# lanl-ansi/GraphicalModelLearning.jl

Measured on AMD Instinct MI355X. Metric: obj/grad evals/sec (RISE, n=1024 spins, 1000000 samples), higher is better.
Workload: dtype i8w

## Files before the change

### graphicalmodellearning.jl_amd/csrc/gml_kernels_i8w.hip

```cpp
#include "gml_i8.h"
#include <string>
#include <type_traits>

namespace gml {

namespace {

constexpr int LFA = 4, LFB = 3;
constexpr int BRT = 32 * LFW;
constexpr int PA = 2 + 2 * LFA, PB = 2 + 2 * LFB;
constexpr int STEPW = PA * 1024, DSW = 2, STAGEW = DSW * STEPW, NSW = 3, RINGW = NSW * STAGEW;
constexpr int NLA = DSW * PA / 4, NLB = DSW * PB / 4;
static_assert(NLA == NLB + 1, "issue() drops the last load in sweep B");

__device__ __forceinline__ double flip_if(double v, int mneg ) {
    return __hiloint2double(__double2hiint(v) + (mneg << 31), __double2loint(v));
}

__device__ __forceinline__ void digits6(double yr, unsigned &dl, unsigned &dh) {
    unsigned long long v = ((unsigned long long)(unsigned)__double2hiint(yr) << 32) | (unsigned)__double2loint(yr);
    v += 0x0000808080808080ull;
    v ^= 0x0000808080808080ull;
    dl = (unsigned)v;
    dh = (unsigned)(v >> 32);
}

__device__ __forceinline__ void dma16(const int8_t *ubase, int voff, unsigned lds_addr) {
    asm volatile("s_mov_b32 m0, %2\n\ts_nop 0\n\tglobal_load_lds_dwordx4 %0, %1" ::"v"(voff), "s"(ubase), "s"(lds_addr) : "memory");
}

}

template <int FORM , bool WANTF, bool WIDE , bool UNIW,
          bool COARSE >
__global__ __launch_bounds__(256, 2) void k_fwd_i8w(
    const unsigned *__restrict__ Xb, const unsigned *__restrict__ Sb, const int8_t *__restrict__ Tq, const int *__restrict__ rowcol,
    const int *__restrict__ groups, int ngroups, const double *__restrict__ w, const double *__restrict__ sigma,
    const long long *__restrict__ qconst, const long long *__restrict__ qconst2, const double *__restrict__ invtau, int64_t Kp, int ntiles_k,
    int nk_all ,
    double wuni, int64_t Kreal, int8_t *__restrict__ Vq, long long *__restrict__ csum, long long *__restrict__ csum2,
    long long *__restrict__ asum, long long *__restrict__ asum2, double *__restrict__ fsum, unsigned *__restrict__ mmax,
    const int *__restrict__ cnk, const int8_t *__restrict__ Xc, int64_t xc_tile, int nk_tq) {
    constexpr int WM = 2;
    extern __shared__ __attribute__((aligned(16))) int8_t lds[];
    double *etab = reinterpret_cast<double *>(lds + RINGW);

    const int tid = threadIdx.x, wave = __builtin_amdgcn_readfirstlane(tid >> 6), lane = tid & 63;
    const int lr = lane & 31, h = lane >> 5;
    if (tid < 64) {
        const double v = exp2((double)tid / 64.0);
        etab[tid] = FORM == 0 ? __hiloint2double(__double2hiint(v) - (tid << 14), __double2loint(v)) : v;
    }
    if (FORM == 2 && tid < 64) {
        const double cj = 1.0 + ((double)tid + 0.5) / 64.0;
        etab[64 + tid] = 1.0 / cj;
        etab[128 + tid] = log(cj);
    }
    __syncthreads();

    constexpr int TG = 8;
    const int b = blockIdx.x, xcd = b & 7, bi = b >> 3;
    const int ntk8 = (ntiles_k + 7) >> 3;
    const int nfull = ngroups / TG, per_full = ntk8 * TG;
    int st, gi;
    if (bi < nfull * per_full) {
        const int rem = bi % per_full;
        st = (rem / TG) * 8 + xcd;
        gi = (bi / per_full) * TG + rem % TG;
    } else {
        const int lastn = ngroups - nfull * TG, rem = bi - nfull * per_full;
        st = (rem / lastn) * 8 + xcd;
        gi = nfull * TG + rem % lastn;
    }
    if (st >= ntiles_k) return;
    const int64_t k0 = (int64_t)st * 256;
    if (k0 >= Kp) return;
    const int mytile = groups[gi];
    int nk = nk_all;
    const int8_t *xbase = reinterpret_cast<const int8_t *>(Xb);
    if (cnk) {
        const int ck = cnk[mytile];
        if (ck >= 0) {
            nk = ck;
            xbase = Xc + (int64_t)mytile * xc_tile;
        }
    }

    const int voffX = lane * 16;
    const int voffT = (lane >> 2) * 64 + (((lane & 3) ^ ((lane >> 4) & 3)) << 4);
    const int8_t *const gX = xbase + (int64_t)(2 * st) * nk * 1024;
    const int8_t *const gT = Tq + (int64_t)mytile * nk_tq * BRT * 64;
    const int nst = (nk + DSW - 1) / DSW;
    const int8_t *baseA[NLA], *baseB[NLB];
    int advA[NLA], advB[NLB], subA[NLA], subB[NLB], dstA[NLA], dstB[NLB];
    bool bitsA[NLA], bitsB[NLB];
    auto plan = [&](int sp, int pps, int row0, const int8_t *&base, int &adv, int &sub, int &dst, bool &bits) {
        sub = sp / pps;
        const int pc = sp - sub * pps;
        dst = sub * STEPW + pc * 1024;
        bits = pc < 2;
        base = bits ? gX + (int64_t)pc * nk * 1024 : gT + (row0 + (pc - 2) * 16) * 64;
        adv = bits ? 1024 : BRT * 64;
    };
#pragma unroll
    for (int j = 0; j < NLA; ++j) plan(wave + 4 * j, PA, 32 * LFB, baseA[j], advA[j], subA[j], dstA[j], bitsA[j]);
#pragma unroll
    for (int j = 0; j < NLB; ++j) plan(wave + 4 * j, PB, 0, baseB[j], advB[j], subB[j], dstB[j], bitsB[j]);
    const unsigned lds0 = (unsigned)(uintptr_t)(__attribute__((address_space(3))) int8_t *)lds;
    auto issue = [&](int gs) {
        const unsigned stage_base = lds0 + (gs % NSW) * STAGEW;
        if (gs < nst) {
#pragma unroll
            for (int j = 0; j < NLA; ++j) {
                int kt = DSW * gs + subA[j];
                kt = kt < nk ? kt : nk - 1;
                dma16(baseA[j] + (int64_t)(kt * advA[j]), bitsA[j] ? voffX : voffT, stage_base + dstA[j]);
            }
        } else {
#pragma unroll
            for (int j = 0; j < NLB; ++j) {
                int kt = DSW * (gs - nst) + subB[j];
                kt = kt < nk ? kt : nk - 1;
                dma16(baseB[j] + (int64_t)(kt * advB[j]), bitsB[j] ? voffX : voffT, stage_base + dstB[j]);
            }
        }
    };

    const int r = mytile * 32 + lr;
    const int rc = rowcol[r];
    const bool active = rc >= 0;
    const double sg = active ? sigma[r] : 0.0;
    const long long qc = active ? (COARSE ? qconst2[r] : qconst[r]) : 0;
    const double c_lo = COARSE ? 0.0 : (double)(unsigned)(qc & 0xffffffll), c_hi = COARSE ? (double)qc : (double)(qc >> 24);
    const double sgT = sg * 16777216.0, us0 = c_hi * sgT, m2sT = -2.0 * sgT;
#ifdef ABL_EARLY_INPUTS
    unsigned sgn[WM];
#pragma unroll
    for (int i = 0; i < WM; ++i) sgn[i] = active ? (Sb[(int64_t)rc * (Kp >> 5) + ((k0 + wave * 64) >> 5) + i] >> (4 * h)) : 0u;
    const double it = active ? invtau[r] : 0.0;
#endif

#ifdef ABL_TIMING
    unsigned long long tst[6];
    tst[0] = __builtin_amdgcn_s_memrealtime();
#endif
    __builtin_amdgcn_s_setprio(1);
    const int ntot = COARSE ? nst : 2 * nst;
#pragma unroll
    for (int s = 0; s < NSW - 1; ++s)
        if (s < ntot) issue(s);
    auto gemm_stage = [&](int gs, int ks, auto first, auto &acc) {
        constexpr bool FIRST = decltype(first)::value;
        constexpr int NPL = sizeof(acc[0]) / sizeof(acc[0][0]);
        if (gs + 1 < ntot) {
            if (gs + 1 < nst) asm volatile("s_waitcnt vmcnt(%0)" ::"n"(NLA) : "memory");
            else asm volatile("s_waitcnt vmcnt(%0)" ::"n"(NLB) : "memory");
        } else {
            asm volatile("s_waitcnt vmcnt(0)" ::: "memory");
        }
        __builtin_amdgcn_s_barrier();
        __builtin_amdgcn_sched_barrier(0);
        if (gs + NSW - 1 < ntot) issue(gs + NSW - 1);
#pragma unroll
        for (int sub = 0; sub < DSW; ++sub) {
            if (sub > 0 && DSW * ks + sub >= nk) break;
            const int8_t *cur = lds + (gs % NSW) * STAGEW + sub * STEPW;
            unsigned vb[WM];
#pragma unroll
            for (int i = 0; i < WM; ++i) {
                const int row = wave * 64 + i * 32 + lr;
                vb[i] = *reinterpret_cast<const unsigned *>(cur + (row >> 7) * 1024 + (((row & 127) * 2 + h) << 2));
            }
#pragma unroll
            for (int t = 0; t < 2; ++t) {
                v4i fa[WM], fb[NPL];
#pragma unroll
                for (int l = 0; l < NPL; ++l) fb[l] = *reinterpret_cast<const v4i *>(cur + 2048 + lds_off(l * 32 + lr, 2 * t + h));
#pragma unroll
                for (int i = 0; i < WM; ++i)
#pragma unroll
                    for (int e = 0; e < 4; ++e) fa[i][e] = (int)((vb[i] >> (4 * t + e)) & 0x01010101u);
#pragma unroll
                for (int i = 0; i < WM; ++i)
#pragma unroll
                    for (int l = 0; l < NPL; ++l) {
                        if (FIRST && sub == 0 && t == 0) acc[i][l] = MFMA_I8(fa[i], fb[l], ((v16i){0, 0, 0, 0, 0, 0, 0, 0, 0, 0, 0, 0, 0, 0, 0, 0}));
                        else acc[i][l] = MFMA_I8(fa[i], fb[l], acc[i][l]);
                    }
            }
        }
    };

    double us[WM][16];
    {
        v16i acc[WM][LFA];
        if (nk > 0) {
            gemm_stage(0, 0, std::true_type{}, acc);
            for (int ks = 1; ks < nst; ++ks) gemm_stage(ks, ks, std::false_type{}, acc);
        } else {
#pragma unroll
            for (int i = 0; i < WM; ++i)
#pragma unroll
                for (int l = 0; l < LFA; ++l)
#pragma unroll
                    for (int e = 0; e < 16; ++e) acc[i][l][e] = 0;
        }
#ifdef ABL_TIMING
        tst[1] = __builtin_amdgcn_s_memrealtime();
#endif
#pragma unroll
        for (int i = 0; i < WM; ++i)
#pragma unroll
            for (int e = 0; e < 16; ++e) {
                double ahi;
                if (WIDE) {
                    ahi = (double)acc[i][3][e];
#pragma unroll
                    for (int l = 2; l >= 0; --l) ahi = fma(ahi, 256.0, (double)acc[i][l][e]);
                } else {
                    const int p0 = acc[i][0][e] + (acc[i][1][e] << 8), p1 = acc[i][2][e] + (acc[i][3][e] << 8);
                    ahi = fma((double)p1, 65536.0, (double)p0);
                }
                us[i][e] = fma(ahi, m2sT, us0);
                asm volatile("" : "+v"(us[i][e]));
            }
    }
#ifdef ABL_TIMING
    tst[2] = __builtin_amdgcn_s_memrealtime();
#endif
    if constexpr (!COARSE) {
        v16i acc[WM][LFB];
        if (nk > 0) {
            gemm_stage(nst, 0, std::true_type{}, acc);
#ifndef ABL_ONESWEEP
            for (int ks = 1; ks < nst; ++ks) gemm_stage(nst + ks, ks, std::false_type{}, acc);
#else
            asm volatile("s_waitcnt vmcnt(0)" ::: "memory");
#endif
        } else {
#pragma unroll
            for (int i = 0; i < WM; ++i)
#pragma unroll
                for (int l = 0; l < LFB; ++l)
#pragma unroll
                    for (int e = 0; e < 16; ++e) acc[i][l][e] = 0;
        }
#pragma unroll
        for (int i = 0; i < WM; ++i)
#pragma unroll
            for (int e = 0; e < 16; ++e) {
                double alo;
                if (WIDE) {
                    alo = fma((double)acc[i][2][e], 256.0, (double)acc[i][1][e]);
                    alo = fma(alo, 256.0, (double)acc[i][0][e]);
                } else {
                    alo = fma((double)acc[i][2][e], 65536.0, (double)(acc[i][0][e] + (acc[i][1][e] << 8)));
                }
                us[i][e] = fma(fma(alo, -2.0, c_lo), sg, us[i][e]);
            }
        __builtin_amdgcn_sched_barrier(0);
    }
    __builtin_amdgcn_s_setprio(0);
#ifdef ABL_TIMING
    tst[3] = __builtin_amdgcn_s_memrealtime();
#endif

#ifndef ABL_EARLY_INPUTS
    unsigned sgn[WM];
#pragma unroll
    for (int i = 0; i < WM; ++i) sgn[i] = active ? (Sb[(int64_t)rc * (Kp >> 5) + ((k0 + wave * 64) >> 5) + i] >> (4 * h)) : 0u;
    const double it = active ? invtau[r] : 0.0;
#endif
    const int64_t left = Kreal - (k0 + wave * 64 + 4 * h);
    const int nreal = left > 64 ? 64 : (left < 0 ? 0 : (int)left);

    int8_t *vimg = Vq + vq_off(mytile * 32 + lr, 0, k0 + wave * 64, Kp, LBW) + h * 32;
    const int64_t kw = k0 + wave * 64;
    const double wscale = COARSE ? 256.0 : 4294967296.0;
    const double wk32 = wscale * (wuni * it);
    const unsigned dh0 = (unsigned)rc * 0x85EBCA6Bu + (unsigned)(kw + 4 * h) * 0x9E3779B9u;
    constexpr double MAGIC = 6755399441055744.0, MAGIC32 = 6755399441055744.0 * 4294967296.0;
    constexpr unsigned GOLD = 0x9E3779B9u;
    const int wleft = (int)((Kreal - kw) < 64 ? (Kreal - kw) : 64);
    int csl[LBW] = {0, 0, 0, 0, 0, 0};
    unsigned long long as64 = 0;
    int ymax_hi = 0;
    double fp = 0.0;

    auto pack4 = [&](const unsigned (&dl)[4], const unsigned (&dhh)[4], v4i (&pl)[LBW], int slot) {
        if (COARSE) {
#pragma unroll
            for (int lb = 0; lb < 3; ++lb) {
                const unsigned sel = ((4u + lb) << 8) | (unsigned)lb;
                const unsigned pk = __builtin_amdgcn_perm(__builtin_amdgcn_perm(dl[3], dl[2], sel), __builtin_amdgcn_perm(dl[1], dl[0], sel), 0x05040100u);
                pl[3 + lb][slot] = (int)pk;
                csl[3 + lb] = __builtin_amdgcn_sdot4((int)pk, 0x01010101, csl[3 + lb], false);
            }
            pl[2][slot] = 0;
            return;
        }
#pragma unroll
        for (int lb = 0; lb < LBW; ++lb) {
            const unsigned bsel = (unsigned)(lb & 3);
            const unsigned sel = ((4u + bsel) << 8) | bsel;
            const unsigned t01 = lb < 4 ? __builtin_amdgcn_perm(dl[1], dl[0], sel) : __builtin_amdgcn_perm(dhh[1], dhh[0], sel);
            const unsigned t23 = lb < 4 ? __builtin_amdgcn_perm(dl[3], dl[2], sel) : __builtin_amdgcn_perm(dhh[3], dhh[2], sel);
            const unsigned pk = __builtin_amdgcn_perm(t23, t01, 0x05040100u);
            pl[lb][slot] = (int)pk;
            csl[lb] = __builtin_amdgcn_sdot4((int)pk, 0x01010101, csl[lb], false);
        }
    };

    if constexpr (FORM == 0) {
#define SB __builtin_amdgcn_sched_barrier(0)
#ifdef I8W_LINE_STORES
        v4i plk[WM][LBW];
#endif
#pragma unroll
        for (int i = 0; i < WM; ++i) {
            const unsigned nsg = ~sgn[i];
            v4i pl[LBW];
#pragma unroll
            for (int hg = 0; hg < 2; ++hg) {
                double Ea[8], tm[8], x[8], tj0[8], yy[8], pp[8], wk[8];
                int mneg[8], nn[8];
#pragma unroll
                for (int q = 0; q < 8; ++q) {
                    const int pos = 8 * (2 * hg + (q >> 2)) + (q & 3);
                    Ea[q] = us[i][8 * hg + q];
                    asm("v_bfe_i32 %0, %1, %2, 1" : "=v"(mneg[q]) : "v"(nsg), "n"(pos));
                    if (!UNIW) wk[q] = w[kw + i * 32 + 8 * (2 * hg + (q >> 2)) + 4 * h + (q & 3)];
                }
                SB;
#ifdef ABL_NOEPI
#pragma unroll
                for (int q = 0; q < 8; ++q) yy[q] = fma(fabs(Ea[q]), 1.0e21, 2.0e23);
                if (false) {
#endif
#pragma unroll
                for (int q = 0; q < 8; ++q) {
                    x[q] = flip_if(Ea[q], mneg[q]);
                    tm[q] = fma(x[q], 92.33248261689366, MAGIC);
                }
                SB;
#pragma unroll
                for (int q = 0; q < 8; ++q) {
                    nn[q] = __double2loint(tm[q]);
                    tm[q] = tm[q] - MAGIC;
                    tj0[q] = etab[nn[q] & 63];
                }
                SB;
#pragma unroll
                for (int q = 0; q < 8; ++q) x[q] = fma(tm[q], -0.01083042469326756, x[q]);
                SB;
#pragma unroll
                for (int q = 0; q < 8; ++q) x[q] = fma(tm[q], -2.9815858269852933e-12, x[q]);
                SB;
#pragma unroll
                for (int q = 0; q < 8; ++q) pp[q] = fma(x[q], 8.3333333333333332e-03, 4.1666666666666664e-02);
                SB;
#pragma unroll
                for (int q = 0; q < 8; ++q) pp[q] = fma(pp[q], x[q], 1.6666666666666666e-01);
                SB;
#pragma unroll
                for (int q = 0; q < 8; ++q) pp[q] = fma(pp[q], x[q], 0.5);
                SB;
#pragma unroll
                for (int q = 0; q < 8; ++q) pp[q] = fma(pp[q], x[q], 1.0);
                SB;
#pragma unroll
                for (int q = 0; q < 8; ++q) pp[q] = pp[q] * x[q];
                SB;
#pragma unroll
                for (int q = 0; q < 8; ++q) {
                    const int idx = i * 32 + 8 * (2 * hg + (q >> 2)) + (q & 3);
                    tj0[q] = __hiloint2double((int)((unsigned)__double2hiint(tj0[q]) + ((unsigned)nn[q] << 14)), __double2loint(tj0[q]));
                    yy[q] = (double)(int)(dh0 + (unsigned)idx * GOLD);
                }
                SB;
#pragma unroll
                for (int q = 0; q < 8; ++q) x[q] = fma(tj0[q], pp[q], tj0[q]);
                SB;
#pragma unroll
                for (int q = 0; q < 8; ++q) yy[q] = fma(UNIW ? wk32 : wscale * (wk[q] * it), x[q], yy[q]);
#ifdef ABL_NOEPI
                }
#endif
                if (UNIW && wleft < 64) {
                    asm volatile("; padding samples" ::: "memory");
#pragma unroll
                    for (int q = 0; q < 8; ++q)
                        if (i * 32 + 8 * (2 * hg + (q >> 2)) + (q & 3) >= nreal) yy[q] = 0.0;
                }
                SB;
#pragma unroll
                for (int q = 0; q < 8; ++q) {
                    ymax_hi = max(ymax_hi, __double2hiint(yy[q]));
                    if (WANTF) {
                        const double ya = yy[q] + MAGIC32;
                        as64 += (((unsigned long long)((unsigned)__double2hiint(ya) & 0xffffu)) << 32) | (unsigned)__double2loint(ya);
                    }
                    x[q] = flip_if(yy[q], mneg[q]) + MAGIC32;
                }
                SB;
#undef SB
#pragma unroll
                for (int gg = 0; gg < 2; ++gg) {
                    unsigned dl[4], dhh[4];
#pragma unroll
                    for (int j = 0; j < 4; ++j) digits6(x[4 * gg + j], dl[j], dhh[j]);
                    pack4(dl, dhh, pl, 2 * hg + gg);
                }
                __builtin_amdgcn_sched_barrier(0);
            }
#ifndef I8W_LINE_STORES
#ifdef ABL_NOSTORE
            if (active && pl[0][0] == 0x12345678 && pl[5][3] == 0x1234567) {
#else
            if (active) {
#endif
#pragma unroll
                for (int lb = COARSE ? 2 : 0; lb < LBW; ++lb) *reinterpret_cast<v4i *>(vimg + lb * 32 * 64 + i * 16) = pl[lb];
            }
#else
#pragma unroll
            for (int lb = COARSE ? 2 : 0; lb < LBW; ++lb) plk[i][lb] = pl[lb];
#endif
        }
#ifdef I8W_LINE_STORES
        {
            const int lastslot = (ntot > 0 ? ntot - 1 : 0) % NSW;
            int8_t *stg = lds + ((lastslot + 1 + (wave >> 1)) % NSW) * STAGEW + (wave & 1) * 6144;
            const unsigned amask = (unsigned)__ballot(active);
            int8_t *img = Vq + vq_off(mytile * 32, 0, kw, Kp, LBW);
            constexpr int G0 = COARSE ? 2 : 0, NG = COARSE ? 2 : 3;
#pragma unroll
            for (int grp = 0; grp < 2; ++grp) {
                const int p0 = G0 + grp * NG;
#pragma unroll
                for (int lbl = 0; lbl < NG; ++lbl)
#pragma unroll
                    for (int i = 0; i < WM; ++i) {
                        const int row = lbl * 32 + lr, sl = 2 * h + i;
                        *reinterpret_cast<v4i *>(stg + row * 64 + ((sl ^ ((row >> 2) & 3)) << 4)) = plk[i][p0 + lbl];
                    }
                asm volatile("s_waitcnt lgkmcnt(0)" ::: "memory");
#pragma unroll
                for (int j = 0; j < 2 * NG; ++j) {
                    const int o = j * 1024 + lane * 16, row = o >> 6, sl = (o >> 4) & 3;
                    const v4i dv = *reinterpret_cast<const v4i *>(stg + row * 64 + ((sl ^ ((row >> 2) & 3)) << 4));
#ifdef ABL_NOSTORE
                    if (dv[0] == 0x12345678 && dv[3] == 0x1234567 && ((amask >> (row & 31)) & 1u))
#else
                    if ((amask >> (row & 31)) & 1u)
#endif
                        *reinterpret_cast<v4i *>(img + p0 * 2048 + o) = dv;
                }
                asm volatile("" ::: "memory");
            }
        }
#endif
    } else {
#pragma unroll
        for (int i = 0; i < WM; ++i) {
            v4i pl[LBW];
#pragma unroll
            for (int g = 0; g < 4; ++g) {
                const int64_t kk = kw + i * 32 + 8 * g + 4 * h;
                unsigned dl[4], dhh[4];
                asm volatile("" : "+v"(fp));
#pragma unroll
                for (int j = 0; j < 4; ++j) {
                    const int e = 4 * g + j;
                    const double Ea = us[i][e];
                    const double dith = (double)(int)(dh0 + (unsigned)(i * 32 + 8 * g + j) * GOLD) * 2.3283064365386963e-10;
                    const bool neg = ((sgn[i] >> (8 * g + j)) & 1u) != 0;
                    const double wk0 = UNIW ? (i * 32 + 8 * g + j < nreal ? wuni : 0.0) : w[kk + j];
                    const double E2 = neg ? -2.0 * Ea : 2.0 * Ea;
                    const double u = exp_tab(-fabs(E2), etab);
                    const double opu = 1.0 + u;
                    double rcp = __builtin_amdgcn_rcp(opu);
                    rcp = fma(fma(-opu, rcp, 1.0), rcp, rcp);
                    rcp = fma(fma(-opu, rcp, 1.0), rcp, rcp);
                    const double sig = E2 >= 0.0 ? u * rcp : rcp;
                    const double y = fma(2.0 * wk0 * it, sig, dith);
                    digits6((neg ? y : -y) + MAGIC, dl[j], dhh[j]);
                    int jt = (int)(u * 64.0);
                    jt = jt > 63 ? 63 : jt;
                    const double r1 = fma(opu, etab[64 + jt], -1.0);
                    double lp = fma(r1, 1.0 / 7.0, -1.0 / 6.0);
                    lp = fma(lp, r1, 0.2);
                    lp = fma(lp, r1, -0.25);
                    lp = fma(lp, r1, 1.0 / 3.0);
                    lp = fma(lp, r1, -0.5);
                    lp = fma(lp, r1, 1.0);
                    const double l1p = fma(lp, r1, etab[128 + jt]);
                    fp += wk0 * ((E2 < 0.0 ? -E2 : 0.0) + l1p);
                }
                pack4(dl, dhh, pl, g);
            }
            if (active) {
#pragma unroll
                for (int lb = 0; lb < LBW; ++lb) *reinterpret_cast<v4i *>(vimg + lb * 32 * 64 + i * 16) = pl[lb];
            }
        }
    }
#ifdef ABL_TIMING
    asm volatile("s_waitcnt vmcnt(0)" ::: "memory");
    tst[4] = __builtin_amdgcn_s_memrealtime();
    if (lane == 0 && wave == 0 && active) {
        unsigned long long *o = reinterpret_cast<unsigned long long *>(Vq + vq_off(mytile * 32, 0, k0, Kp, LBW));
        for (int q = 0; q < 5; ++q) o[q] = tst[q];
        o[5] = (unsigned long long)__builtin_amdgcn_s_getreg((4 << 0) | (0 << 6) | (31 << 11)) ;
    }
#endif
    long long cs_lo = (long long)csl[0] + 256ll * csl[1] + 65536ll * csl[2];
    long long cs_hi = (long long)csl[3] + 256ll * csl[4] + 65536ll * csl[5];
    cs_lo += __shfl_xor(cs_lo, 32);
    cs_hi += __shfl_xor(cs_hi, 32);
    if (active && h == 0) {
        if (!COARSE) atomicAdd(reinterpret_cast<unsigned long long *>(&csum[r]), (unsigned long long)cs_lo);
        atomicAdd(reinterpret_cast<unsigned long long *>(&csum2[r]), (unsigned long long)cs_hi);
    }
    if (FORM == 0) {
        if (WANTF) {
            as64 += __shfl_xor(as64, 32);
            if (active && h == 0) {
                atomicAdd(reinterpret_cast<unsigned long long *>(&asum[r]), as64 & 0xffffffffull);
                atomicAdd(reinterpret_cast<unsigned long long *>(&asum2[r]), as64 >> 32);
            }
        }
        ymax_hi = max(ymax_hi, __shfl_xor(ymax_hi, 32));
        const double ymax = __hiloint2double(ymax_hi + 1, 0);
        const unsigned mxu = COARSE ? (((unsigned)fmin(ymax * 2.3283064365386963e-10 , 8388606.0) + 1u) << 8)
                                    : (unsigned)fmin(ymax * 3.5527136788005009e-15 , 4294967295.0);
        if (active && h == 0) atomicMax(&mmax[r], mxu);
    } else {
        fp += __shfl_xor(fp, 32);
        if (active && h == 0) unsafeAtomicAdd(&fsum[r], fp);
    }
}

__global__ __launch_bounds__(256) void k_finalize_i8w(const int32_t *__restrict__ Gacc, const double *__restrict__ tau,
                                                      const long long *__restrict__ csum, const long long *__restrict__ csum2,
                                                      const long long *__restrict__ asum, const long long *__restrict__ asum2,
                                                      const int *__restrict__ srow, const int *__restrict__ rowcol, int slot0, int64_t Qp,
                                                      int64_t Qfp, int64_t Qf, int64_t cconst, int form, int want_grad,
                                                      double *__restrict__ G, double *__restrict__ f, int nplanes, int64_t plane_stride,
                                                      const unsigned *__restrict__ mmax, SlotResult *__restrict__ res,
                                                      int coarse ) {
    const int r = slot0 + blockIdx.y;
    if (rowcol[r] < 0) return;
    const int64_t c = (int64_t)blockIdx.x * 256 + threadIdx.x;
    const double t = tau[r];
    const int tile = r >> 5, rl = r & 31;
    auto gcol = [&](int64_t col) -> double {
        long long s[2] = {0, 0};
#pragma unroll
        for (int half = 0; half < 2; ++half) {
            if (coarse && half == 0) continue;
#pragma unroll
            for (int l = 2; l >= 0; --l) {
                long long a = 0;
                for (int pl = 0; pl < nplanes; ++pl) a += (long long)Gacc[pl * plane_stride + ((int64_t)(tile * LBW + 3 * half + l) * 32 + rl) * Qfp + col];
                s[half] = s[half] * 256 + a;
            }
        }
        return fma((double)(csum2[r] - 2 * s[1]), 16777216.0, coarse ? 0.0 : (double)(csum[r] - 2 * s[0]));
    };
    if (c == 0) {
        double fv = f ? f[r] : 0.0;
        if (form != 2) {
            if (want_grad) fv = -t * gcol(rowcol[r]);
            else fv = t * (coarse ? 16777216.0 : 1.0) * fma((double)asum2[r], 4294967296.0, (double)asum[r]);
            f[r] = fv;
        }
        if (res) res[r] = SlotResult{fv, t, mmax[r], 0u};
    }
    if (!want_grad || c >= Qp) return;
    double v = 0.0;
    if (c < Qf) v = t * gcol(c);
    else if (c == cconst) v = t * fma((double)csum2[r], 16777216.0, coarse ? 0.0 : (double)csum[r]);
    G[(int64_t)srow[r] * Qp + c] = v;
}

void launch_finalize_i8w(const int32_t *Gacc, const SlotScalars &sc, const int *srow, const int *rowcol, int slot0, int ns, int64_t Qp,
                         int64_t Qfp, int64_t Qf, int64_t cconst, int form, int want_grad, double *G, double *f, int nplanes,
                         int64_t plane_stride, SlotResult *res, bool coarse, hipStream_t st) {
    hipLaunchKernelGGL(k_finalize_i8w, dim3((unsigned)((Qp + 255) / 256), (unsigned)ns), dim3(256), 0, st, Gacc, sc.tau, sc.csum, sc.csum2,
                       sc.asum, sc.asum2, srow, rowcol, slot0, Qp, Qfp, Qf, cconst, form, want_grad, G, f, nplanes, plane_stride, sc.mmax, res,
                       coarse ? 1 : 0);
}

template <int FORM, bool WANTF, bool WIDE, bool UNIW, bool COARSE>
static void launch_fwd_w5(const FwdWArgs &a) {
    constexpr int shmem = RINGW + 512 + 1024;
    (void)hipFuncSetAttribute(reinterpret_cast<const void *>(&k_fwd_i8w<FORM, WANTF, WIDE, UNIW, COARSE>),
                              hipFuncAttributeMaxDynamicSharedMemorySize, shmem);
    const DevProblem &d = *a.d;
    const int ntk = (int)(d.Kp / 256);
    const int grid = ((ntk + 7) / 8) * 8 * a.ngroups;
    hipLaunchKernelGGL((k_fwd_i8w<FORM, WANTF, WIDE, UNIW, COARSE>), dim3(grid), dim3(256), shmem, a.st, d.Xb, d.Sb, a.Tq, a.rowcol, a.groups,
                       a.ngroups, d.w, a.sc->sigma, a.sc->qconst, a.sc->qconst2, a.sc->invtau, d.Kp, ntk, a.zero_theta ? 0 : (int)(d.Qfp / 64), d.wuni, d.K, a.Vq,
                       a.sc->csum, a.sc->csum2, a.sc->asum, a.sc->asum2, a.F, a.sc->mmax, a.cc ? a.cc->cnk : nullptr, a.cc ? a.cc->Xc : nullptr,
                       a.cc ? a.cc->xc_tile : 0, (int)(d.Qfp / 64));
}

template <int FORM, bool WANTF, bool WIDE, bool UNIW>
static void launch_fwd_w4(const FwdWArgs &a) {
    if constexpr (FORM == 0) {
        if (a.coarse) return launch_fwd_w5<FORM, WANTF, WIDE, UNIW, true>(a);
    }
    launch_fwd_w5<FORM, WANTF, WIDE, UNIW, false>(a);
}

template <int FORM, bool WANTF, bool WIDE>
static void launch_fwd_w3(const FwdWArgs &a) {
    if (a.d->wuni > 0.0) launch_fwd_w4<FORM, WANTF, WIDE, true>(a);
    else launch_fwd_w4<FORM, WANTF, WIDE, false>(a);
}

template <int FORM, bool WANTF>
static void launch_fwd_w2(const FwdWArgs &a) {
    if (a.d->Qfp > 32768) launch_fwd_w3<FORM, WANTF, true>(a);
    else launch_fwd_w3<FORM, WANTF, false>(a);
}

void launch_fwd_i8w(const FwdWArgs &a) {
    if (a.form == 2) launch_fwd_w2<2, true>(a);
    else if (a.want_f) launch_fwd_w2<0, true>(a);
    else launch_fwd_w2<0, false>(a);
}

}
```

### graphicalmodellearning.jl_amd/csrc/gml_testhooks.cpp

```cpp
#include "gml_internal.h"
#include "gml_solver.h"
#include "gml_pack.h"

#include <algorithm>
#include <atomic>
#include <chrono>
#include <cmath>
#include <cstdarg>
#include <cstdio>
#include <cstdlib>
#include <cstring>
#include <condition_variable>
#include <mutex>
#include <thread>

using namespace gml;

namespace gml {
double g_hv_sparse_ratio = 0.3;
std::atomic<long long> g_hv_sparse_calls{0};
double g_tune[GML_NTUNE] = {};
}
extern "C" long long gml_test_hv_sparse_calls(void) { return g_hv_sparse_calls.load(); }
extern "C" double gml_test_tune(int id, double value) {
    if (id < 0 || id >= GML_NTUNE) return NAN;
    const double old = g_tune[id];
    g_tune[id] = value;
    return old;
}
extern "C" double gml_test_hv_sparse_ratio(double ratio) {
    const double old = g_hv_sparse_ratio;
    g_hv_sparse_ratio = ratio;
    return old;
}


extern "C" int gml_test_tile_precond(int T, int ntiles, const int *m, const double *tiles , double s1, double s2,
                                     const double *g , const double *r , double *z_out ,
                                     int device) {
    if ((T != 64 && T != 128) || ntiles <= 0) return fail(GML_EINVAL, "bad tile size");
    HIPCHK(hipSetDevice(device));
    const size_t nt = (size_t)ntiles, ne = nt * T;
    std::vector<long long> hoff(nt);
    std::vector<int> wrow(nt, 0), fv(ne), live(1, 1);
    for (size_t t = 0; t < nt; ++t) hoff[t] = (long long)t * T * T;
    for (size_t e = 0; e < ne; ++e) fv[e] = (int)e;
    double *dH = nullptr, *dS1 = nullptr, *dG = nullptr, *dR = nullptr, *dZ = nullptr;
    long long *dHoff = nullptr;
    int *dM = nullptr, *dWrow = nullptr, *dFv = nullptr, *dLive = nullptr;
    auto freeall = [&]() {
        void *ptrs[] = {dH, dS1, dG, dR, dZ, dHoff, dM, dWrow, dFv, dLive};
        for (void *q : ptrs)
            if (q) (void)dev_free(q);
    };
#define TCHK2(expr)                                                                              \
    do {                                                                                        \
        if ((expr) != hipSuccess) {                                                             \
            freeall();                                                                          \
            return fail(GML_EHIP, "%s failed: %s", #expr, hipGetErrorString(hipGetLastError())); \
        }                                                                                       \
    } while (0)
    TCHK2(dev_malloc(&dH, sizeof(double) * ne * T));
    TCHK2(dev_malloc(&dS1, sizeof(double)));
    TCHK2(dev_malloc(&dG, sizeof(double) * ne));
    TCHK2(dev_malloc(&dR, sizeof(double) * ne));
    TCHK2(dev_malloc(&dZ, sizeof(double) * ne));
    TCHK2(dev_malloc(&dHoff, sizeof(long long) * nt));
    TCHK2(dev_malloc(&dM, sizeof(int) * nt));
    TCHK2(dev_malloc(&dWrow, sizeof(int) * nt));
    TCHK2(dev_malloc(&dFv, sizeof(int) * ne));
    TCHK2(dev_malloc(&dLive, sizeof(int)));
    TCHK2(hipMemcpy(dH, tiles, sizeof(double) * ne * T, hipMemcpyHostToDevice));
    TCHK2(hipMemcpy(dS1, &s1, sizeof(double), hipMemcpyHostToDevice));
    TCHK2(hipMemcpy(dG, g, sizeof(double) * ne, hipMemcpyHostToDevice));
    TCHK2(hipMemcpy(dR, r, sizeof(double) * ne, hipMemcpyHostToDevice));
    TCHK2(hipMemset(dZ, 0, sizeof(double) * ne));
    TCHK2(hipMemcpy(dHoff, hoff.data(), sizeof(long long) * nt, hipMemcpyHostToDevice));
    TCHK2(hipMemcpy(dM, m, sizeof(int) * nt, hipMemcpyHostToDevice));
    TCHK2(hipMemcpy(dWrow, wrow.data(), sizeof(int) * nt, hipMemcpyHostToDevice));
    TCHK2(hipMemcpy(dFv, fv.data(), sizeof(int) * ne, hipMemcpyHostToDevice));
    TCHK2(hipMemcpy(dLive, live.data(), sizeof(int), hipMemcpyHostToDevice));
    launch_tile_inverse(T, dH, dHoff, dM, dWrow, dS1, s2, dG, ntiles, nullptr);
    launch_tile_apply(T, dH, dFv, dM, dWrow, dLive, ntiles, (int64_t)ne, dR, dZ, nullptr);
    TCHK2(hipGetLastError());
    TCHK2(hipDeviceSynchronize());
    TCHK2(hipMemcpy(z_out, dZ, sizeof(double) * ne, hipMemcpyDeviceToHost));
#undef TCHK2
    freeall();
    return GML_OK;
}

static int test_newton_solve(int R, const int *m, int cap, const double *blocks, const double *pg, double s2, const double *g, double *d_out,
                             int device, const unsigned char *fix , const double *dfix ) {
    HIPCHK(hipSetDevice(device));
    std::vector<long long> hoff((size_t)R + 1, 0);
    std::vector<int> mt((size_t)R);
    int maxm = 0;
    for (int r = 0; r < R; ++r) {
        if (m[r] < 0 || m[r] > cap || cap > 512) return fail(GML_EINVAL, "bad block size");
        mt[r] = (m[r] + 31) / 32;
        hoff[r + 1] = hoff[r] + (long long)mt[r] * 32 * mt[r] * 32;
        maxm = std::max(maxm, m[r]);
    }
    std::vector<double> H((size_t)std::max<long long>(hoff[R], 1), 0.0), s1((size_t)R, 1.0), gz((size_t)R * cap, 0.0);
    for (int r = 0; r < R; ++r) {
        const int hp = 32 * mt[r];
        for (int i = 0; i < m[r]; ++i)
            for (int j = 0; j < m[r]; ++j) H[(size_t)hoff[r] + (size_t)i * hp + j] = blocks[((size_t)r * cap + i) * cap + j];
        for (int i = m[r]; i < hp; ++i) H[(size_t)hoff[r] + (size_t)i * hp + i] = 1.0;
    }
    double *dH = nullptr, *dS1 = nullptr, *dG = nullptr, *dPg = nullptr, *dOut = nullptr, *dSd = nullptr, *dDfix = nullptr;
    long long *dHoff = nullptr;
    int *dMt = nullptr, *dM = nullptr, *dRedo = nullptr;
    uint8_t *dFix = nullptr;
    auto freeall = [&]() {
        void *ptrs[] = {dH, dS1, dG, dPg, dOut, dSd, dHoff, dMt, dM, dDfix, dRedo, dFix};
        for (void *q : ptrs)
            if (q) (void)dev_free(q);
    };
#define TCHK(expr)                                                           \
    do {                                                                     \
        if ((expr) != hipSuccess) {                                          \
            freeall();                                                       \
            return fail(GML_EHIP, "%s failed: %s", #expr, hipGetErrorString(hipGetLastError())); \
        }                                                                    \
    } while (0)
    TCHK(dev_malloc(&dH, sizeof(double) * H.size()));
    TCHK(dev_malloc(&dS1, sizeof(double) * R));
    TCHK(dev_malloc(&dG, sizeof(double) * R * cap));
    TCHK(dev_malloc(&dPg, sizeof(double) * R * cap));
    TCHK(dev_malloc(&dOut, sizeof(double) * R * cap));
    TCHK(dev_malloc(&dSd, sizeof(double) * R));
    TCHK(dev_malloc(&dHoff, sizeof(long long) * (R + 1)));
    TCHK(dev_malloc(&dMt, sizeof(int) * R));
    TCHK(dev_malloc(&dM, sizeof(int) * R));
    TCHK(hipMemcpy(dH, H.data(), sizeof(double) * H.size(), hipMemcpyHostToDevice));
    TCHK(hipMemcpy(dS1, s1.data(), sizeof(double) * R, hipMemcpyHostToDevice));
    TCHK(hipMemcpy(dG, g ? g : gz.data(), sizeof(double) * R * cap, hipMemcpyHostToDevice));
    TCHK(hipMemcpy(dPg, pg, sizeof(double) * R * cap, hipMemcpyHostToDevice));
    TCHK(hipMemcpy(dHoff, hoff.data(), sizeof(long long) * (R + 1), hipMemcpyHostToDevice));
    TCHK(hipMemcpy(dMt, mt.data(), sizeof(int) * R, hipMemcpyHostToDevice));
    TCHK(hipMemcpy(dM, m, sizeof(int) * R, hipMemcpyHostToDevice));
    TCHK(hipMemset(dOut, 0, sizeof(double) * R * cap));
    if (fix) {
        TCHK(dev_malloc(&dFix, (size_t)R * cap));
        TCHK(dev_malloc(&dDfix, sizeof(double) * R * cap));
        TCHK(hipMemcpy(dFix, fix, (size_t)R * cap, hipMemcpyHostToDevice));
        TCHK(hipMemcpy(dDfix, dfix, sizeof(double) * R * cap, hipMemcpyHostToDevice));
    }
    launch_newton_solve(dH, dHoff, dMt, dM, dS1, s2, dG, dPg, R, cap, dOut, dSd, nullptr, maxm, nullptr, dFix, dDfix);
    TCHK(hipGetLastError());
    TCHK(hipDeviceSynchronize());
    TCHK(hipMemcpy(d_out, dOut, sizeof(double) * R * cap, hipMemcpyDeviceToHost));
#undef TCHK
    freeall();
    return GML_OK;
}

extern "C" int gml_test_newton_solve(int R, const int *m, int cap, const double *blocks ,
                                     const double *pg , double s2, const double *g , double *d_out ,
                                     int device) {
    return test_newton_solve(R, m, cap, blocks, pg, s2, g, d_out, device, nullptr, nullptr);
}
extern "C" int gml_test_newton_solve_fixed(int R, const int *m, int cap, const double *blocks, const double *pg, double s2, const double *g,
                                           const unsigned char *fix, const double *dfix, double *d_out, int device) {
    return test_newton_solve(R, m, cap, blocks, pg, s2, g, d_out, device, fix, dfix);
}

extern "C" int gml_debug_read_vq(gml_problem *p, int64_t off, int64_t bytes, void *out) {
    if (!p || !out) return fail(GML_EINVAL, "NULL argument");
    HIPCHK(hipSetDevice(p->device));
    const int8_t *vq = nullptr;
    int64_t total = 0;
    gml::i8_vq_buffer(p->i8ws, &vq, &total, p->d);
    if (!vq || off < 0 || off + bytes > total) return fail(GML_EINVAL, "range outside the %lld bytes of V planes", (long long)total);
    HIPCHK(hipStreamSynchronize(p->st));
    HIPCHK(hipMemcpy(out, vq + off, (size_t)bytes, hipMemcpyDeviceToHost));
    return GML_OK;
}
```

Before: 97270.

## Fuse the two i8w GEMM sweeps into one pass over all weight planes

Adds a one-sweep path to the i8 forward kernel, made the default for non-coarse forms. Each k-step now loads the two X bit planes and all LFW theta planes into a 4-stage LDS ring and accumulates all seven planes at once. Previously the kernel ran two separate sweeps (LFA then LFB planes), which read X twice. This halves X traffic and barrier count, at the cost of more accumulator registers (WM*LFW v16i), possible occupancy pressure, and a different ring size. Wide FORM 2 and coarse modes keep the old two-sweep path, and a test hook is added.

```diff
diff --git a/graphicalmodellearning.jl_amd/csrc/gml_kernels_i8w.hip b/graphicalmodellearning.jl_amd/csrc/gml_kernels_i8w.hip
--- a/graphicalmodellearning.jl_amd/csrc/gml_kernels_i8w.hip
+++ b/graphicalmodellearning.jl_amd/csrc/gml_kernels_i8w.hip
@@ -12,6 +12,18 @@
 constexpr int STEPW = PA * 1024, DSW = 2, STAGEW = DSW * STEPW, NSW = 3, RINGW = NSW * STAGEW;
 constexpr int NLA = DSW * PA / 4, NLB = DSW * PB / 4;
 static_assert(NLA == NLB + 1, "issue() drops the last load in sweep B");
+constexpr int P1 = 2 + 2 * LFW, STEP1 = P1 * 1024, NS1 = 4, RING1 = NS1 * STEP1, NL1 = P1 / 4;
+static_assert(P1 % 4 == 0 && NL1 == 4, "one stage: 4 DMA instructions per wave");
+#ifdef I8W_TWO_SWEEPS
+constexpr bool ONE_SWEEP = false;
+#else
+constexpr bool ONE_SWEEP = true;
+#endif
+#if defined(I8W_LINE_STORES) && !defined(I8W_TWO_SWEEPS)
+#error "I8W_LINE_STORES stages through the ring of the two-sweep form: build it with -DI8W_TWO_SWEEPS"
+#endif
+constexpr bool one_sweep(int form, bool wide, bool coarse) { return ONE_SWEEP && !coarse && !(form == 2 && wide); }
+constexpr int ring_bytes(int form, bool wide, bool coarse) { return one_sweep(form, wide, coarse) ? RING1 : RINGW; }
 
 __device__ __forceinline__ double flip_if(double v, int mneg ) {
     return __hiloint2double(__double2hiint(v) + (mneg << 31), __double2loint(v));
@@ -43,10 +55,10 @@
     const int *__restrict__ cnk, const int8_t *__restrict__ Xc, int64_t xc_tile, int nk_tq) {
     constexpr int WM = 2;
     extern __shared__ __attribute__((aligned(16))) int8_t lds[];
-    double *etab = reinterpret_cast<double *>(lds + RINGW);
-
-    const int tid = threadIdx.x, wave = __builtin_amdgcn_readfirstlane(tid >> 6), lane = tid & 63;
-    const int lr = lane & 31, h = lane >> 5;
+    double *etab = reinterpret_cast<double *>(lds + ring_bytes(FORM, WIDE, COARSE));
+
+    const int tid = threadIdx.x, wave = __builtin_amdgcn_readfirstlane(tid >> 6);
+    int lane = tid & 63, lr = lane & 31, h = lane >> 5;
     if (tid < 64) {
         const double v = exp2((double)tid / 64.0);
         etab[tid] = FORM == 0 ? __hiloint2double(__double2hiint(v) - (tid << 14), __double2loint(v)) : v;
@@ -90,49 +102,10 @@
     const int voffT = (lane >> 2) * 64 + (((lane & 3) ^ ((lane >> 4) & 3)) << 4);
     const int8_t *const gX = xbase + (int64_t)(2 * st) * nk * 1024;
     const int8_t *const gT = Tq + (int64_t)mytile * nk_tq * BRT * 64;
-    const int nst = (nk + DSW - 1) / DSW;
-    const int8_t *baseA[NLA], *baseB[NLB];
-    int advA[NLA], advB[NLB], subA[NLA], subB[NLB], dstA[NLA], dstB[NLB];
-    bool bitsA[NLA], bitsB[NLB];
-    auto plan = [&](int sp, int pps, int row0, const int8_t *&base, int &adv, int &sub, int &dst, bool &bits) {
-        sub = sp / pps;
-        const int pc = sp - sub * pps;
-        dst = sub * STEPW + pc * 1024;
-        bits = pc < 2;
-        base = bits ? gX + (int64_t)pc * nk * 1024 : gT + (row0 + (pc - 2) * 16) * 64;
-        adv = bits ? 1024 : BRT * 64;
-    };
-#pragma unroll
-    for (int j = 0; j < NLA; ++j) plan(wave + 4 * j, PA, 32 * LFB, baseA[j], advA[j], subA[j], dstA[j], bitsA[j]);
-#pragma unroll
-    for (int j = 0; j < NLB; ++j) plan(wave + 4 * j, PB, 0, baseB[j], advB[j], subB[j], dstB[j], bitsB[j]);
     const unsigned lds0 = (unsigned)(uintptr_t)(__attribute__((address_space(3))) int8_t *)lds;
-    auto issue = [&](int gs) {
-        const unsigned stage_base = lds0 + (gs % NSW) * STAGEW;
-        if (gs < nst) {
-#pragma unroll
-            for (int j = 0; j < NLA; ++j) {
-                int kt = DSW * gs + subA[j];
-                kt = kt < nk ? kt : nk - 1;
-                dma16(baseA[j] + (int64_t)(kt * advA[j]), bitsA[j] ? voffX : voffT, stage_base + dstA[j]);
-            }
-        } else {
-#pragma unroll
-            for (int j = 0; j < NLB; ++j) {
-                int kt = DSW * (gs - nst) + subB[j];
-                kt = kt < nk ? kt : nk - 1;
-                dma16(baseB[j] + (int64_t)(kt * advB[j]), bitsB[j] ? voffX : voffT, stage_base + dstB[j]);
-            }
-        }
-    };
-
-    const int r = mytile * 32 + lr;
+    int r = mytile * 32 + lr;
     const int rc = rowcol[r];
     const bool active = rc >= 0;
-    const double sg = active ? sigma[r] : 0.0;
-    const long long qc = active ? (COARSE ? qconst2[r] : qconst[r]) : 0;
-    const double c_lo = COARSE ? 0.0 : (double)(unsigned)(qc & 0xffffffll), c_hi = COARSE ? (double)qc : (double)(qc >> 24);
-    const double sgT = sg * 16777216.0, us0 = c_hi * sgT, m2sT = -2.0 * sgT;
 #ifdef ABL_EARLY_INPUTS
     unsigned sgn[WM];
 #pragma unroll
@@ -144,121 +117,259 @@
     unsigned long long tst[6];
     tst[0] = __builtin_amdgcn_s_memrealtime();
 #endif
-    __builtin_amdgcn_s_setprio(1);
-    const int ntot = COARSE ? nst : 2 * nst;
-#pragma unroll
-    for (int s = 0; s < NSW - 1; ++s)
-        if (s < ntot) issue(s);
-    auto gemm_stage = [&](int gs, int ks, auto first, auto &acc) {
-        constexpr bool FIRST = decltype(first)::value;
-        constexpr int NPL = sizeof(acc[0]) / sizeof(acc[0][0]);
-        if (gs + 1 < ntot) {
-            if (gs + 1 < nst) asm volatile("s_waitcnt vmcnt(%0)" ::"n"(NLA) : "memory");
-            else asm volatile("s_waitcnt vmcnt(%0)" ::"n"(NLB) : "memory");
-        } else {
-            asm volatile("s_waitcnt vmcnt(0)" ::: "memory");
-        }
-        __builtin_amdgcn_s_barrier();
-        __builtin_amdgcn_sched_barrier(0);
-        if (gs + NSW - 1 < ntot) issue(gs + NSW - 1);
-#pragma unroll
-        for (int sub = 0; sub < DSW; ++sub) {
-            if (sub > 0 && DSW * ks + sub >= nk) break;
-            const int8_t *cur = lds + (gs % NSW) * STAGEW + sub * STEPW;
+    double us[WM][16];
+    if constexpr (one_sweep(FORM, WIDE, COARSE)) {
+        const int8_t *base1[NL1];
+        int adv1[NL1];
+#pragma unroll
+        for (int j = 0; j < NL1; ++j) {
+            const int pc = wave + 4 * j;
+            base1[j] = pc < 2 ? gX + (int64_t)pc * nk * 1024 : gT + (pc - 2) * 16 * 64;
+            adv1[j] = pc < 2 ? 1024 : BRT * 64;
+        }
+        const int voff0 = wave < 2 ? voffX : voffT;
+        auto issue1 = [&](int ks) {
+            const unsigned stage_base = lds0 + (ks % NS1) * STEP1;
+#pragma unroll
+            for (int j = 0; j < NL1; ++j) dma16(base1[j] + (int64_t)ks * adv1[j], j == 0 ? voff0 : voffT, stage_base + (wave + 4 * j) * 1024);
+        };
+        __builtin_amdgcn_s_setprio(1);
+#pragma unroll
+        for (int s = 0; s < NS1 - 1; ++s)
+            if (s < nk) issue1(s);
+        v16i acc[WM][LFW];
+        auto step = [&](int ks, auto first) {
+            constexpr bool FIRST = decltype(first)::value;
+            if (ks + 2 < nk) asm volatile("s_waitcnt vmcnt(%0)" ::"n"(2 * NL1) : "memory");
+            else if (ks + 1 < nk) asm volatile("s_waitcnt vmcnt(%0)" ::"n"(NL1) : "memory");
+            else asm volatile("s_waitcnt vmcnt(0)" ::: "memory");
+            __builtin_amdgcn_s_barrier();
+            __builtin_amdgcn_sched_barrier(0);
+            if (ks + NS1 - 1 < nk) issue1(ks + NS1 - 1);
+            const int8_t *cur = lds + (ks % NS1) * STEP1;
             unsigned vb[WM];
 #pragma unroll
             for (int i = 0; i < WM; ++i) {
                 const int row = wave * 64 + i * 32 + lr;
-                vb[i] = *reinterpret_cast<const unsigned *>(cur + (row >> 7) * 1024 + (((row & 127) * 2 + h) << 2));
+                const uint2 v = *reinterpret_cast<const uint2 *>(cur + (row >> 7) * 1024 + (row & 127) * 8);
+                vb[i] = h ? v.y : v.x;
             }
 #pragma unroll
             for (int t = 0; t < 2; ++t) {
-                v4i fa[WM], fb[NPL];
-#pragma unroll
-                for (int l = 0; l < NPL; ++l) fb[l] = *reinterpret_cast<const v4i *>(cur + 2048 + lds_off(l * 32 + lr, 2 * t + h));
+                v4i fa[WM];
 #pragma unroll
                 for (int i = 0; i < WM; ++i)
 #pragma unroll
                     for (int e = 0; e < 4; ++e) fa[i][e] = (int)((vb[i] >> (4 * t + e)) & 0x01010101u);
 #pragma unroll
-                for (int i = 0; i < WM; ++i)
-#pragma unroll
-                    for (int l = 0; l < NPL; ++l) {
-                        if (FIRST && sub == 0 && t == 0) acc[i][l] = MFMA_I8(fa[i], fb[l], ((v16i){0, 0, 0, 0, 0, 0, 0, 0, 0, 0, 0, 0, 0, 0, 0, 0}));
-                        else acc[i][l] = MFMA_I8(fa[i], fb[l], acc[i][l]);
+                for (int l = 0; l < LFW; ++l) {
+                    const v4i fb = *reinterpret_cast<const v4i *>(cur + 2048 + lds_off(l * 32 + lr, 2 * t + h));
+#pragma unroll
+                    for (int i = 0; i < WM; ++i) {
+                        if (FIRST && t == 0) acc[i][l] = MFMA_I8(fa[i], fb, ((v16i){0, 0, 0, 0, 0, 0, 0, 0, 0, 0, 0, 0, 0, 0, 0, 0}));
+                        else acc[i][l] = MFMA_I8(fa[i], fb, acc[i][l]);
                     }
-            }
-        }
-    };
-
-    double us[WM][16];
-    {
-        v16i acc[WM][LFA];
+                }
+            }
+        };
         if (nk > 0) {
-            gemm_stage(0, 0, std::true_type{}, acc);
-            for (int ks = 1; ks < nst; ++ks) gemm_stage(ks, ks, std::false_type{}, acc);
+            step(0, std::true_type{});
+            for (int ks = 1; ks < nk; ++ks) step(ks, std::false_type{});
         } else {
 #pragma unroll
             for (int i = 0; i < WM; ++i)
 #pragma unroll
-                for (int l = 0; l < LFA; ++l)
+                for (int l = 0; l < LFW; ++l)
 #pragma unroll
                     for (int e = 0; e < 16; ++e) acc[i][l][e] = 0;
         }
 #ifdef ABL_TIMING
-        tst[1] = __builtin_amdgcn_s_memrealtime();
-#endif
+        tst[1] = tst[2] = __builtin_amdgcn_s_memrealtime();
+#endif
+        lane = __lane_id();
+        lr = lane & 31;
+        h = lane >> 5;
+        r = mytile * 32 + lr;
+        const double sg = active ? sigma[r] : 0.0;
+        const long long qc = active ? qconst[r] : 0;
+        const double c_lo = (double)(unsigned)(qc & 0xffffffll), c_hi = (double)(qc >> 24);
+        const double sgT = sg * 16777216.0, us0 = c_hi * sgT, m2sT = -2.0 * sgT;
 #pragma unroll
         for (int i = 0; i < WM; ++i)
 #pragma unroll
             for (int e = 0; e < 16; ++e) {
-                double ahi;
+                double ahi, alo;
                 if (WIDE) {
-                    ahi = (double)acc[i][3][e];
-#pragma unroll
-                    for (int l = 2; l >= 0; --l) ahi = fma(ahi, 256.0, (double)acc[i][l][e]);
-                } else {
-                    const int p0 = acc[i][0][e] + (acc[i][1][e] << 8), p1 = acc[i][2][e] + (acc[i][3][e] << 8);
-                    ahi = fma((double)p1, 65536.0, (double)p0);
-                }
-                us[i][e] = fma(ahi, m2sT, us0);
-                asm volatile("" : "+v"(us[i][e]));
-            }
-    }
-#ifdef ABL_TIMING
-    tst[2] = __builtin_amdgcn_s_memrealtime();
-#endif
-    if constexpr (!COARSE) {
-        v16i acc[WM][LFB];
-        if (nk > 0) {
-            gemm_stage(nst, 0, std::true_type{}, acc);
-#ifndef ABL_ONESWEEP
-            for (int ks = 1; ks < nst; ++ks) gemm_stage(nst + ks, ks, std::false_type{}, acc);
-#else
-            asm volatile("s_waitcnt vmcnt(0)" ::: "memory");
-#endif
-        } else {
-#pragma unroll
-            for (int i = 0; i < WM; ++i)
-#pragma unroll
-                for (int l = 0; l < LFB; ++l)
-#pragma unroll
-                    for (int e = 0; e < 16; ++e) acc[i][l][e] = 0;
-        }
-#pragma unroll
-        for (int i = 0; i < WM; ++i)
-#pragma unroll
-            for (int e = 0; e < 16; ++e) {
-                double alo;
-                if (WIDE) {
+                    ahi = (double)acc[i][6][e];
+#pragma unroll
+                    for (int l = 5; l >= 3; --l) ahi = fma(ahi, 256.0, (double)acc[i][l][e]);
                     alo = fma((double)acc[i][2][e], 256.0, (double)acc[i][1][e]);
                     alo = fma(alo, 256.0, (double)acc[i][0][e]);
                 } else {
+                    const int p0 = acc[i][3][e] + (acc[i][4][e] << 8), p1 = acc[i][5][e] + (acc[i][6][e] << 8);
+                    ahi = fma((double)p1, 65536.0, (double)p0);
                     alo = fma((double)acc[i][2][e], 65536.0, (double)(acc[i][0][e] + (acc[i][1][e] << 8)));
                 }
-                us[i][e] = fma(fma(alo, -2.0, c_lo), sg, us[i][e]);
+                us[i][e] = fma(fma(alo, -2.0, c_lo), sg, fma(ahi, m2sT, us0));
+                asm volatile("" : "+v"(us[i][e]));
             }
         __builtin_amdgcn_sched_barrier(0);
+    } else {
+        const int nst = (nk + DSW - 1) / DSW;
+        const int8_t *baseA[NLA], *baseB[NLB];
+        int advA[NLA], advB[NLB], subA[NLA], subB[NLB], dstA[NLA], dstB[NLB];
+        bool bitsA[NLA], bitsB[NLB];
+        auto plan = [&](int sp, int pps, int row0, const int8_t *&base, int &adv, int &sub, int &dst, bool &bits) {
+            sub = sp / pps;
+            const int pc = sp - sub * pps;
+            dst = sub * STEPW + pc * 1024;
+            bits = pc < 2;
+            base = bits ? gX + (int64_t)pc * nk * 1024 : gT + (row0 + (pc - 2) * 16) * 64;
+            adv = bits ? 1024 : BRT * 64;
+        };
+#pragma unroll
+        for (int j = 0; j < NLA; ++j) plan(wave + 4 * j, PA, 32 * LFB, baseA[j], advA[j], subA[j], dstA[j], bitsA[j]);
+#pragma unroll
+        for (int j = 0; j < NLB; ++j) plan(wave + 4 * j, PB, 0, baseB[j], advB[j], subB[j], dstB[j], bitsB[j]);
+        auto issue = [&](int gs) {
+            const unsigned stage_base = lds0 + (gs % NSW) * STAGEW;
+            if (gs < nst) {
+#pragma unroll
+                for (int j = 0; j < NLA; ++j) {
+                    int kt = DSW * gs + subA[j];
+                    kt = kt < nk ? kt : nk - 1;
+                    dma16(baseA[j] + (int64_t)(kt * advA[j]), bitsA[j] ? voffX : voffT, stage_base + dstA[j]);
+                }
+            } else {
+#pragma unroll
+                for (int j = 0; j < NLB; ++j) {
+                    int kt = DSW * (gs - nst) + subB[j];
+                    kt = kt < nk ? kt : nk - 1;
+                    dma16(baseB[j] + (int64_t)(kt * advB[j]), bitsB[j] ? voffX : voffT, stage_base + dstB[j]);
+                }
+            }
+        };
+
+        const double sg = active ? sigma[r] : 0.0;
+        const long long qc = active ? (COARSE ? qconst2[r] : qconst[r]) : 0;
+        const double c_lo = COARSE ? 0.0 : (double)(unsigned)(qc & 0xffffffll), c_hi = COARSE ? (double)qc : (double)(qc >> 24);
+        const double sgT = sg * 16777216.0, us0 = c_hi * sgT, m2sT = -2.0 * sgT;
+
+        __builtin_amdgcn_s_setprio(1);
+        const int ntot = COARSE ? nst : 2 * nst;
+#pragma unroll
+        for (int s = 0; s < NSW - 1; ++s)
+            if (s < ntot) issue(s);
+        auto gemm_stage = [&](int gs, int ks, auto first, auto &acc) {
+            constexpr bool FIRST = decltype(first)::value;
+            constexpr int NPL = sizeof(acc[0]) / sizeof(acc[0][0]);
+            if (gs + 1 < ntot) {
+                if (gs + 1 < nst) asm volatile("s_waitcnt vmcnt(%0)" ::"n"(NLA) : "memory");
+                else asm volatile("s_waitcnt vmcnt(%0)" ::"n"(NLB) : "memory");
+            } else {
+                asm volatile("s_waitcnt vmcnt(0)" ::: "memory");
+            }
+            __builtin_amdgcn_s_barrier();
+            __builtin_amdgcn_sched_barrier(0);
+            if (gs + NSW - 1 < ntot) issue(gs + NSW - 1);
+#pragma unroll
+            for (int sub = 0; sub < DSW; ++sub) {
+                if (sub > 0 && DSW * ks + sub >= nk) break;
+                const int8_t *cur = lds + (gs % NSW) * STAGEW + sub * STEPW;
+                unsigned vb[WM];
+#pragma unroll
+                for (int i = 0; i < WM; ++i) {
+                    const int row = wave * 64 + i * 32 + lr;
+                    vb[i] = *reinterpret_cast<const unsigned *>(cur + (row >> 7) * 1024 + (((row & 127) * 2 + h) << 2));
+                }
+#pragma unroll
+                for (int t = 0; t < 2; ++t) {
+                    v4i fa[WM], fb[NPL];
+#pragma unroll
+                    for (int l = 0; l < NPL; ++l) fb[l] = *reinterpret_cast<const v4i *>(cur + 2048 + lds_off(l * 32 + lr, 2 * t + h));
+#pragma unroll
+                    for (int i = 0; i < WM; ++i)
+#pragma unroll
+                        for (int e = 0; e < 4; ++e) fa[i][e] = (int)((vb[i] >> (4 * t + e)) & 0x01010101u);
+#pragma unroll
+                    for (int i = 0; i < WM; ++i)
+#pragma unroll
+                        for (int l = 0; l < NPL; ++l) {
+                            if (FIRST && sub == 0 && t == 0) acc[i][l] = MFMA_I8(fa[i], fb[l], ((v16i){0, 0, 0, 0, 0, 0, 0, 0, 0, 0, 0, 0, 0, 0, 0, 0}));
+                            else acc[i][l] = MFMA_I8(fa[i], fb[l], acc[i][l]);
+                        }
+                }
+            }
+        };
+
+        {
+            v16i acc[WM][LFA];
+            if (nk > 0) {
+                gemm_stage(0, 0, std::true_type{}, acc);
+                for (int ks = 1; ks < nst; ++ks) gemm_stage(ks, ks, std::false_type{}, acc);
+            } else {
+#pragma unroll
+                for (int i = 0; i < WM; ++i)
+#pragma unroll
+                    for (int l = 0; l < LFA; ++l)
+#pragma unroll
+                        for (int e = 0; e < 16; ++e) acc[i][l][e] = 0;
+            }
+#ifdef ABL_TIMING
+            tst[1] = __builtin_amdgcn_s_memrealtime();
+#endif
+#pragma unroll
+            for (int i = 0; i < WM; ++i)
+#pragma unroll
+                for (int e = 0; e < 16; ++e) {
+                    double ahi;
+                    if (WIDE) {
+                        ahi = (double)acc[i][3][e];
+#pragma unroll
+                        for (int l = 2; l >= 0; --l) ahi = fma(ahi, 256.0, (double)acc[i][l][e]);
+                    } else {
+                        const int p0 = acc[i][0][e] + (acc[i][1][e] << 8), p1 = acc[i][2][e] + (acc[i][3][e] << 8);
+                        ahi = fma((double)p1, 65536.0, (double)p0);
+                    }
+                    us[i][e] = fma(ahi, m2sT, us0);
+                    asm volatile("" : "+v"(us[i][e]));
+                }
+        }
+#ifdef ABL_TIMING
+        tst[2] = __builtin_amdgcn_s_memrealtime();
+#endif
+        if constexpr (!COARSE) {
+            v16i acc[WM][LFB];
+            if (nk > 0) {
+                gemm_stage(nst, 0, std::true_type{}, acc);
+#ifndef ABL_ONESWEEP
+                for (int ks = 1; ks < nst; ++ks) gemm_stage(nst + ks, ks, std::false_type{}, acc);
+#else
+                asm volatile("s_waitcnt vmcnt(0)" ::: "memory");
+#endif
+            } else {
+#pragma unroll
+                for (int i = 0; i < WM; ++i)
+#pragma unroll
+                    for (int l = 0; l < LFB; ++l)
+#pragma unroll
+                        for (int e = 0; e < 16; ++e) acc[i][l][e] = 0;
+            }
+#pragma unroll
+            for (int i = 0; i < WM; ++i)
+#pragma unroll
+                for (int e = 0; e < 16; ++e) {
+                    double alo;
+                    if (WIDE) {
+                        alo = fma((double)acc[i][2][e], 256.0, (double)acc[i][1][e]);
+                        alo = fma(alo, 256.0, (double)acc[i][0][e]);
+                    } else {
+                        alo = fma((double)acc[i][2][e], 65536.0, (double)(acc[i][0][e] + (acc[i][1][e] << 8)));
+                    }
+                    us[i][e] = fma(fma(alo, -2.0, c_lo), sg, us[i][e]);
+                }
+            __builtin_amdgcn_sched_barrier(0);
+        }
     }
     __builtin_amdgcn_s_setprio(0);
 #ifdef ABL_TIMING
@@ -429,6 +540,7 @@
         }
 #ifdef I8W_LINE_STORES
         {
+            const int nst = (nk + DSW - 1) / DSW, ntot = COARSE ? nst : 2 * nst;
             const int lastslot = (ntot > 0 ? ntot - 1 : 0) % NSW;
             int8_t *stg = lds + ((lastslot + 1 + (wave >> 1)) % NSW) * STAGEW + (wave & 1) * 6144;
             const unsigned amask = (unsigned)__ballot(active);
@@ -594,7 +706,7 @@
 
 template <int FORM, bool WANTF, bool WIDE, bool UNIW, bool COARSE>
 static void launch_fwd_w5(const FwdWArgs &a) {
-    constexpr int shmem = RINGW + 512 + 1024;
+    constexpr int shmem = ring_bytes(FORM, WIDE, COARSE) + 512 + 1024;
     (void)hipFuncSetAttribute(reinterpret_cast<const void *>(&k_fwd_i8w<FORM, WANTF, WIDE, UNIW, COARSE>),
                               hipFuncAttributeMaxDynamicSharedMemorySize, shmem);
     const DevProblem &d = *a.d;
diff --git a/graphicalmodellearning.jl_amd/csrc/gml_testhooks.cpp b/graphicalmodellearning.jl_amd/csrc/gml_testhooks.cpp
--- a/graphicalmodellearning.jl_amd/csrc/gml_testhooks.cpp
+++ b/graphicalmodellearning.jl_amd/csrc/gml_testhooks.cpp
@@ -1,4 +1,5 @@
 #include "gml_internal.h"
+#include "gml_i8.h"
 #include "gml_solver.h"
 #include "gml_pack.h"
 
@@ -178,3 +179,24 @@
     HIPCHK(hipMemcpy(out, vq + off, (size_t)bytes, hipMemcpyDeviceToHost));
     return GML_OK;
 }
+
+
+extern "C" int gml_test_i8_pass_state(gml_problem *p, int64_t *slots, int *planes, int64_t *kp, int8_t *vq, long long *sums) {
+    if (!p || !slots || !planes || !kp) return fail(GML_EINVAL, "bad argument");
+    const gml::I8Ws *w = static_cast<const gml::I8Ws *>(p->i8ws);
+    *slots = w ? w->slots : 0;
+    *planes = w ? w->LBT : 0;
+    *kp = p->d.Kp;
+    if (!w || !vq || !sums) return GML_OK;
+    HIPCHK(hipSetDevice(p->device));
+    HIPCHK(hipStreamSynchronize(p->st));
+    const size_t ns = (size_t)w->slots;
+    HIPCHK(hipMemcpy(vq, w->Vq, ns * w->LBT * p->d.Kp, hipMemcpyDeviceToHost));
+    const gml::SlotScalars &sc = w->sc[0];
+    const long long *src[4] = {sc.csum, sc.csum2, sc.asum, sc.asum2};
+    for (int j = 0; j < 4; ++j) HIPCHK(hipMemcpy(sums + j * ns, src[j], sizeof(long long) * ns, hipMemcpyDeviceToHost));
+    std::vector<unsigned> mm(ns);
+    HIPCHK(hipMemcpy(mm.data(), sc.mmax, sizeof(unsigned) * ns, hipMemcpyDeviceToHost));
+    for (size_t i = 0; i < ns; ++i) sums[4 * ns + i] = mm[i];
+    return GML_OK;
+}
```

Measured after the change: 101,700 (median of 6 runs). 4.5% higher.
